# mpizenberg/visual-odometry-rs

Measured on AMD Instinct MI355X. Metric: frame-pairs/sec (640x480, 6 pyramid levels), higher is better.
Workload: dtype f32

## Files before the change

visual-odometry-rs_amd/csrc/kernels.hip:

```cpp
#include <hip/hip_runtime.h>

#include <algorithm>
#include <cstdint>
#include <cstdlib>

#include "device_common.h"
#include "engine.h"
#include "synth_scene.h"

namespace vors {

template <class T>
__global__ void transpose_kernel(const T* __restrict__ src, T* __restrict__ dst, int rows, int cols) {
    __shared__ T tile[32][33];
    const size_t base = (size_t)blockIdx.z * rows * cols;
    int sx = blockIdx.x * 32 + threadIdx.x;
    int sy = blockIdx.y * 32 + threadIdx.y;
    for (int j = 0; j < 32; j += 8)
        if (sx < rows && sy + j < cols) tile[threadIdx.y + j][threadIdx.x] = src[base + (size_t)(sy + j) * rows + sx];
    __syncthreads();
    int dx = blockIdx.y * 32 + threadIdx.x;
    int dy = blockIdx.x * 32 + threadIdx.y;
    for (int j = 0; j < 32; j += 8)
        if (dx < cols && dy + j < rows) dst[base + (size_t)(dy + j) * cols + dx] = tile[threadIdx.x][threadIdx.y + j];
// ... 315 lines not shown
                uint32_t k3 = (uint32_t)__builtin_amdgcn_update_dpp(0, (int)key, 0xff, 0xf, 0xf, true);
                {
                    uint32_t lo, hi;
                    lo = min(k0, k1); hi = max(k0, k1); k0 = lo; k1 = hi;
                    lo = min(k2, k3); hi = max(k2, k3); k2 = lo; k3 = hi;
                    lo = min(k0, k2); hi = max(k0, k2); k0 = lo; k2 = hi;
                    lo = min(k1, k3); hi = max(k1, k3); k1 = lo; k3 = hi;
                    lo = min(k1, k2); hi = max(k1, k2); k1 = lo; k2 = hi;
                }
                const uint32_t second = k2 >> 2, third = k1 >> 2;
                const bool keep2 = second > ((third + thresh) & 0xffffu);
                if (in && key >= k2) {
                    const bool best = key == k3;
                    const int dst = rl * NODES + offc + 2 * k + (best ? 0 : 1);
                    xy[dst] = (pvalid && (best || keep2)) ? ((uint32_t)cx | ((uint32_t)cy << 16)) : VORS_INVALID_XY;
                    gr[dst] = slim_pack_tg(tm, gx, gy);
                }
            }
        }
        kf_wave_sync();
    }

    {
        const int cap = 1 << (L - 1), off = cap - 1;
        for (int t = lane; t < KF_R * cap; t += 64) {
            const int rl = t >> (L - 1), k = t & (cap - 1);
            const uint32_t p = xy[rl * NODES + off + k];
            if (p != VORS_INVALID_XY) {
                const uint16_t dz = (depth + (size_t)pair * g.S0)[(p >> 16) * (unsigned)g.lv[0].cols + (p & 0xffffu)];
                if (dz == 0) {
                    xy[rl * NODES + off + k] = VORS_INVALID_XY;
                } else {
                    sd[rl * NODES + off + k] = g.depth_scale / (float)dz;
                    sv[rl * NODES + off + k] = g.idepth_variance;
                }
            }
        }
    }
    kf_wave_sync();
#pragma unroll
    for (int l = 1; l < L; ++l) {
        const int cap = 1 << (L - 1 - l);
        const int off = cap - 1, offc = 2 * cap - 1;
        for (int t = lane; t < KF_R * cap; t += 64) {
            const int rl = t >> (L - 1 - l), k = t & (cap - 1);
            const int c1 = rl * NODES + offc + 2 * k, c2 = c1 + 1, dst = rl * NODES + off + k;
            const bool k1 = xy[c1] != VORS_INVALID_XY, k2 = xy[c2] != VORS_INVALID_XY;
            if (k1 && k2) {
                const float d1 = sd[c1], v1 = sv[c1], d2 = sd[c2], v2 = sv[c2];
                const float sum = v1 + v2;
                sd[dst] = (d1 * v1 + d2 * v2) / sum;
                sv[dst] = sum;
            } else if (k1 || k2) {
                const int src = k1 ? c1 : c2;
                sd[dst] = sd[src];
                sv[dst] = sv[src];
            } else {
                xy[dst] = VORS_INVALID_XY;
            }
        }
        kf_wave_sync();
    }
    const int region = blockIdx.x * KF_WAVES + wave;
#pragma unroll
    for (int l = 0; l < L; ++l) {
        const int cap = 1 << (L - 1 - l), off = cap - 1;
        const int n_here = min(KF_R, max(0, n_roots - root0)) * cap;
        SlimRec* out = rec.stage + (size_t)pair * g.slots_total + g.lv[l].slot_off + (size_t)root0 * cap;
        int filled = 0;
        for (int base = 0; base < n_here; base += 64) {
            const int t = base + lane;
            const int rl = t >> (L - 1 - l), k = t & (cap - 1);
            const bool in = t < n_here;
            const uint32_t p = in ? xy[rl * NODES + off + k] : VORS_INVALID_XY;
            const bool valid = p != VORS_INVALID_XY;
            const unsigned long long m = __ballot(valid);
            const int before = __builtin_amdgcn_mbcnt_hi((unsigned)(m >> 32), __builtin_amdgcn_mbcnt_lo((unsigned)m, 0));
            if (valid) out[(unsigned)(filled + before)] = SlimRec{p, sd[rl * NODES + off + k], gr[rl * NODES + off + k]};
            filled += __popcll(m);
        }
        if (lane == 0) rec.region_cnt[((size_t)pair * VORS_MAX_LEVELS + l) * rec.n_regions + region] = filled;
    }
}

__global__ __launch_bounds__(256) void compact_regions_kernel(Geom g, Records rec) {
    __shared__ int s_cnt[256], s_pre[256], s_wave[4];
    __shared__ int s_base;
    const int pair = select_pair(g, blockIdx.y);
    if (pair < 0) return;
    const int lane = threadIdx.x & 63, wave = threadIdx.x >> 6;
    const int l_first = gridDim.x > 1 ? (int)blockIdx.x : 0, l_end = gridDim.x > 1 ? l_first + 1 : g.L;
    for (int l = l_first; l < l_end; ++l) {
        const int cap_r = rec.kf_r << (g.L - 1 - l);
        const int* cnt = rec.region_cnt + ((size_t)pair * VORS_MAX_LEVELS + l) * rec.n_regions;
        const size_t lvl0 = (size_t)pair * g.slots_total + g.lv[l].slot_off;
        const SlimRec* src = rec.stage + lvl0;
        SlimRec* dst = rec.S + lvl0;
        __syncthreads();
        if (threadIdx.x == 0) s_base = 0;
        __syncthreads();
        for (int tile = 0; tile < rec.n_regions; tile += 256) {
            const int r = tile + (int)threadIdx.x;
            const int mine = r < rec.n_regions ? cnt[r] : 0;
            int incl = mine;
#pragma unroll
            for (int o = 1; o < 64; o <<= 1) {
                const int v = __shfl_up(incl, o);
                if (lane >= o) incl += v;
            }
            if (lane == 63) s_wave[wave] = incl;
            __syncthreads();
            int pre = s_base + incl - mine;
            for (int w = 0; w < wave; ++w) pre += s_wave[w];
            s_cnt[threadIdx.x] = mine;
            s_pre[threadIdx.x] = pre;
            __syncthreads();
            const int n_tile = min(256, rec.n_regions - tile);
            const int cap_sh = __ffs(cap_r) - 1;
            for (int j = threadIdx.x; j < n_tile * cap_r; j += 256) {
                const int rr = j >> cap_sh, k = j & (cap_r - 1);
                if (k < s_cnt[rr]) dst[s_pre[rr] + k] = src[(size_t)(tile + rr) * cap_r + k];
            }
            __syncthreads();
            if (threadIdx.x == 255) s_base = pre + mine;
            __syncthreads();
        }
        if (threadIdx.x == 0) rec.n_used[(size_t)pair * VORS_MAX_LEVELS + l] = s_base;
    }
}

__device__ __forceinline__ void fuse_dso_mean(const float dv_in[4], const float vv_in[4], float* od, float* ov) {
    float sd = 0.f, sv = 0.f, single = 0.f;
    int n = 0;
#pragma unroll
    for (int m = 0; m < 4; ++m) {
        const bool known = vv_in[m] >= 0.f;
        const float prod = dv_in[m] * vv_in[m];
        sd += known ? prod : 0.f;
        sv += known ? vv_in[m] : 0.f;
        single = known ? dv_in[m] : single;
        n += known ? 1 : 0;
    }
    const float q = sd / sv;
    *od = n == 0 ? __builtin_nanf("") : (n == 1 ? single : q);
    *ov = n == 0 ? -1.0f : sv;
}
template <bool FAST>
__device__ __forceinline__ float idepth_of(float scale, uint32_t dz) {
    const float d = (float)dz;
    if (FAST) {
        const float rc = __builtin_amdgcn_rcpf(d);
        const float q = scale * rc;
        return fmaf(fmaf(-q, d, scale), rc, q);
    }
    return scale / d;
}
template <bool FAST>
__device__ __forceinline__ void fuse_depths(float scale, float var, const uint32_t dz[4], float* od, float* ov, int& n0) {
    float sd = 0.f, sv = 0.f, s1 = 0.f;
    int n = 0;
#pragma unroll
    for (int m = 0; m < 4; ++m) {
        const bool known = dz[m] != 0;
        const float d = known ? idepth_of<FAST>(scale, dz[m]) : 0.f;
        sd += d * var;
        sv += known ? var : 0.f;
        s1 += d;
        n += known ? 1 : 0;
    }
    n0 += n;
    const float q = sd / sv;
    *od = n == 0 ? __builtin_nanf("") : (n == 1 ? s1 : q);
    *ov = n == 0 ? -1.0f : sv;
}
__global__ void verify_idepth_kernel(float scale, int* mismatch) {
    const uint32_t dz = blockIdx.x * blockDim.x + threadIdx.x;
    if (dz == 0 || dz > 65535u) return;
    if (idepth_of<true>(scale, dz) != idepth_of<false>(scale, dz)) atomicExch(mismatch, 1);
}
bool verify_fast_idepth(float scale, hipStream_t s) {
    if (!(scale == scale) || !(fabsf(scale) < 1e30f) || !(fabsf(scale) > 1e-20f)) return false;
    int* flag = nullptr;
    if (hipMalloc(reinterpret_cast<void**>(&flag), sizeof(int)) != hipSuccess) return false;
    (void)hipMemsetAsync(flag, 0, sizeof(int), s);
    hipLaunchKernelGGL(verify_idepth_kernel, dim3(256), dim3(256), 0, s, scale, flag);
    int h = 1;
    const bool ok = hipMemcpyAsync(&h, flag, sizeof(int), hipMemcpyDeviceToHost, s) == hipSuccess && hipStreamSynchronize(s) == hipSuccess;
    (void)hipFree(flag);
    return ok && h == 0;
}
__device__ __forceinline__ void count_add(int* counter, int n) {
#pragma unroll
    for (int o = 32; o >= 1; o >>= 1) n += __shfl_xor(n, o);
    if ((threadIdx.x & 63) == 0 && n != 0) atomicAdd(counter, n);
}
template <bool FAST>
__global__ __launch_bounds__(256) void dense_idepth_level1_kernel(Geom g, const uint16_t* __restrict__ depth, Records rec) {
    const int pair = select_pair(g, blockIdx.y);
    if (pair < 0) return;
    const int t = blockIdx.x * blockDim.x + threadIdx.x;
    const int rows = g.lv[1].rows, cols = g.lv[1].cols;
    int n0 = 0, n1 = 0;
    if (t < rows * cols) {
        const int y = t / cols, x = t - y * cols;
        const int fr = g.lv[0].rows, fc = g.lv[0].cols;
        const uint16_t* p = depth + (size_t)pair * g.S0 + (size_t)(2 * y) * fc + 2 * x;
        const uint32_t dz[4] = {p[0], p[fc], p[1], p[fc + 1]};
        float od, ov;
        fuse_depths<FAST>(g.depth_scale, g.idepth_variance, dz, &od, &ov, n0);
        const bool last_x = x == cols - 1 && (fc & 1), last_y = y == rows - 1 && (fr & 1);
        if (last_x) n0 += (p[2] != 0) + (p[fc + 2] != 0);
        if (last_y) n0 += (p[2 * fc] != 0) + (p[2 * fc + 1] != 0);
        if (last_x && last_y) n0 += p[2 * fc + 2] != 0;
        const size_t slot = (size_t)pair * g.slots_total + g.lv[1].slot_off + t;
        rec.IZ[slot] = od;
        rec.V[slot] = ov;
        n1 = ov >= 0.f;
    }
    count_add(rec.n_used + (size_t)pair * VORS_MAX_LEVELS + 0, n0);
    count_add(rec.n_used + (size_t)pair * VORS_MAX_LEVELS + 1, n1);
}
template <bool FAST>
__global__ __launch_bounds__(256) void dense_idepth_level1_wide_kernel(Geom g, const uint16_t* __restrict__ depth, Records rec) {
    const int pair = select_pair(g, blockIdx.y);
    if (pair < 0) return;
    const int t0 = (blockIdx.x * blockDim.x + threadIdx.x) * 4;
    const int rows = g.lv[1].rows, cols = g.lv[1].cols;
    int n0 = 0, n1 = 0;
    if (t0 < rows * cols) {
        const int y = t0 / cols, x0 = t0 - y * cols;
        const int fr = g.lv[0].rows, fc = g.lv[0].cols;
        const uint16_t* p = depth + (size_t)pair * g.S0 + (size_t)(2 * y) * fc + 2 * x0;
        const uint4 r0 = *reinterpret_cast<const uint4*>(p), r1 = *reinterpret_cast<const uint4*>(p + fc);
        const uint32_t w0[4] = {r0.x, r0.y, r0.z, r0.w}, w1[4] = {r1.x, r1.y, r1.z, r1.w};
        float od[4], ov[4];
#pragma unroll
        for (int k = 0; k < 4; ++k) {
            const uint32_t dz[4] = {w0[k] & 0xffffu, w1[k] & 0xffffu, w0[k] >> 16, w1[k] >> 16};
            fuse_depths<FAST>(g.depth_scale, g.idepth_variance, dz, &od[k], &ov[k], n0);
            n1 += ov[k] >= 0.f;
        }
        if (y == rows - 1 && (fr & 1)) {
            const uint4 r2 = *reinterpret_cast<const uint4*>(p + 2 * fc);
            const uint32_t w2[4] = {r2.x, r2.y, r2.z, r2.w};
#pragma unroll
            for (int k = 0; k < 4; ++k) n0 += ((w2[k] & 0xffffu) != 0) + ((w2[k] >> 16) != 0);
        }
        const size_t slot = (size_t)pair * g.slots_total + g.lv[1].slot_off + t0;
        *reinterpret_cast<float4*>(rec.IZ + slot) = make_float4(od[0], od[1], od[2], od[3]);
        *reinterpret_cast<float4*>(rec.V + slot) = make_float4(ov[0], ov[1], ov[2], ov[3]);
    }
    count_add(rec.n_used + (size_t)pair * VORS_MAX_LEVELS + 0, n0);
    count_add(rec.n_used + (size_t)pair * VORS_MAX_LEVELS + 1, n1);
}
template <bool FAST>
__global__ __launch_bounds__(256) void dense_idepth_level12_kernel(Geom g, const uint16_t* __restrict__ depth, Records rec) {
    const int pair = select_pair(g, blockIdx.y);
    if (pair < 0) return;
    const int t = (blockIdx.x * blockDim.x + threadIdx.x) * 2;
    const int rows2 = g.lv[2].rows, cols2 = g.lv[2].cols;
    int n0 = 0, n1 = 0, n2 = 0;
    if (t < rows2 * cols2) {
        const int y2 = t / cols2, x2 = t - y2 * cols2;
        const int fc = g.lv[0].cols, c1 = g.lv[1].cols;
        const uint16_t* p = depth + (size_t)pair * g.S0 + (size_t)(4 * y2) * fc + 4 * x2;
        uint32_t w[4][4];
#pragma unroll
        for (int r = 0; r < 4; ++r) {
            const uint4 v = *reinterpret_cast<const uint4*>(p + (size_t)r * fc);
            w[r][0] = v.x;
            w[r][1] = v.y;
            w[r][2] = v.z;
            w[r][3] = v.w;
        }
        float od1[2][4], ov1[2][4];
#pragma unroll
        for (int i = 0; i < 2; ++i)
#pragma unroll
            for (int j = 0; j < 4; ++j) {
                const uint32_t top = w[2 * i][j], bot = w[2 * i + 1][j];
                const uint32_t dz[4] = {top & 0xffffu, bot & 0xffffu, top >> 16, bot >> 16};
                fuse_depths<FAST>(g.depth_scale, g.idepth_variance, dz, &od1[i][j], &ov1[i][j], n0);
                n1 += ov1[i][j] >= 0.f;
            }
        const size_t s1 = (size_t)pair * g.slots_total + g.lv[1].slot_off + (size_t)(2 * y2) * c1 + 2 * x2;
        *reinterpret_cast<float4*>(rec.IZ + s1) = make_float4(od1[0][0], od1[0][1], od1[0][2], od1[0][3]);
        *reinterpret_cast<float4*>(rec.IZ + s1 + c1) = make_float4(od1[1][0], od1[1][1], od1[1][2], od1[1][3]);
        float od[2], ov[2];
#pragma unroll
        for (int k = 0; k < 2; ++k) {
            const float dv2[4] = {od1[0][2 * k], od1[1][2 * k], od1[0][2 * k + 1], od1[1][2 * k + 1]};
            const float vv2[4] = {ov1[0][2 * k], ov1[1][2 * k], ov1[0][2 * k + 1], ov1[1][2 * k + 1]};
            fuse_dso_mean(dv2, vv2, &od[k], &ov[k]);
            n2 += ov[k] >= 0.f;
        }
        const size_t s2 = (size_t)pair * g.slots_total + g.lv[2].slot_off + t;
        *reinterpret_cast<float2*>(rec.IZ + s2) = make_float2(od[0], od[1]);
        *reinterpret_cast<float2*>(rec.V + s2) = make_float2(ov[0], ov[1]);
    }
    count_add(rec.n_used + (size_t)pair * VORS_MAX_LEVELS + 0, n0);
    count_add(rec.n_used + (size_t)pair * VORS_MAX_LEVELS + 1, n1);
    count_add(rec.n_used + (size_t)pair * VORS_MAX_LEVELS + 2, n2);
}
template <bool FAST>
__global__ __launch_bounds__(256) void dense_idepth_level123_kernel(Geom g, const uint16_t* __restrict__ depth, Records rec) {
    const int pair = select_pair(g, blockIdx.y);
    if (pair < 0) return;
    const int t = blockIdx.x * blockDim.x + threadIdx.x;
    const int cols3 = g.lv[3].cols;
    int n0 = 0, n1 = 0, n2 = 0, n3 = 0;
    if (t < g.lv[3].rows * cols3) {
        const int y3 = t / cols3, x3 = t - y3 * cols3;
        const int fc = g.lv[0].cols, c1 = g.lv[1].cols, c2 = g.lv[2].cols;
        const size_t base = (size_t)pair * g.slots_total;
        float od2[2][2], ov2[2][2];
        const uint16_t* p = depth + (size_t)pair * g.S0 + (size_t)(8 * y3) * fc + 8 * x3;
        uint4 v8[8];
#pragma unroll
        for (int r = 0; r < 8; ++r) v8[r] = *reinterpret_cast<const uint4*>(p + (size_t)r * fc);
#pragma unroll
        for (int h = 0; h < 2; ++h) {
            uint32_t w[4][4];
#pragma unroll
            for (int r = 0; r < 4; ++r) {
                const uint4 v = v8[4 * h + r];
                w[r][0] = v.x;
                w[r][1] = v.y;
                w[r][2] = v.z;
                w[r][3] = v.w;
            }
            float od1[2][4], ov1[2][4];
#pragma unroll
            for (int i = 0; i < 2; ++i)
#pragma unroll
                for (int j = 0; j < 4; ++j) {
                    const uint32_t top = w[2 * i][j], bot = w[2 * i + 1][j];
                    const uint32_t dz[4] = {top & 0xffffu, bot & 0xffffu, top >> 16, bot >> 16};
                    fuse_depths<FAST>(g.depth_scale, g.idepth_variance, dz, &od1[i][j], &ov1[i][j], n0);
                    n1 += ov1[i][j] >= 0.f;
                }
            const size_t s1 = base + g.lv[1].slot_off + (size_t)(4 * y3 + 2 * h) * c1 + 4 * x3;
            *reinterpret_cast<float4*>(rec.IZ + s1) = make_float4(od1[0][0], od1[0][1], od1[0][2], od1[0][3]);
            *reinterpret_cast<float4*>(rec.IZ + s1 + c1) = make_float4(od1[1][0], od1[1][1], od1[1][2], od1[1][3]);
#pragma unroll
            for (int k = 0; k < 2; ++k) {
                const float dv[4] = {od1[0][2 * k], od1[1][2 * k], od1[0][2 * k + 1], od1[1][2 * k + 1]};
                const float vv[4] = {ov1[0][2 * k], ov1[1][2 * k], ov1[0][2 * k + 1], ov1[1][2 * k + 1]};
                fuse_dso_mean(dv, vv, &od2[h][k], &ov2[h][k]);
                n2 += ov2[h][k] >= 0.f;
            }
            const size_t s2 = base + g.lv[2].slot_off + (size_t)(2 * y3 + h) * c2 + 2 * x3;
            *reinterpret_cast<float2*>(rec.IZ + s2) = make_float2(od2[h][0], od2[h][1]);
            *reinterpret_cast<float2*>(rec.V + s2) = make_float2(ov2[h][0], ov2[h][1]);
        }
        const float dv[4] = {od2[0][0], od2[1][0], od2[0][1], od2[1][1]};
        const float vv[4] = {ov2[0][0], ov2[1][0], ov2[0][1], ov2[1][1]};
        float od, ov;
        fuse_dso_mean(dv, vv, &od, &ov);
        n3 = ov >= 0.f;
        const size_t s3 = base + g.lv[3].slot_off + t;
        rec.IZ[s3] = od;
        rec.V[s3] = ov;
    }
    count_add(rec.n_used + (size_t)pair * VORS_MAX_LEVELS + 0, n0);
    count_add(rec.n_used + (size_t)pair * VORS_MAX_LEVELS + 1, n1);
    count_add(rec.n_used + (size_t)pair * VORS_MAX_LEVELS + 2, n2);
    count_add(rec.n_used + (size_t)pair * VORS_MAX_LEVELS + 3, n3);
}
__global__ __launch_bounds__(256) void dense_idepth_halve_kernel(Geom g, int l, Records rec) {
    const int pair = select_pair(g, blockIdx.y);
    if (pair < 0) return;
    const int t = blockIdx.x * blockDim.x + threadIdx.x;
    const int rows = g.lv[l].rows, cols = g.lv[l].cols;
    int n = 0;
    if (t < rows * cols) {
        const int y = t / cols, x = t - y * cols;
        const int fc = g.lv[l - 1].cols;
        const size_t cb = (size_t)pair * g.slots_total + g.lv[l - 1].slot_off + (size_t)(2 * y) * fc + 2 * x;
        const size_t idx[4] = {cb, cb + fc, cb + 1, cb + fc + 1};
        float dv[4], vv[4];
#pragma unroll
        for (int m = 0; m < 4; ++m) {
            dv[m] = rec.IZ[idx[m]];
            vv[m] = rec.V[idx[m]];
        }
        float od, ov;
        fuse_dso_mean(dv, vv, &od, &ov);
        const size_t slot = (size_t)pair * g.slots_total + g.lv[l].slot_off + t;
        rec.IZ[slot] = od;
        rec.V[slot] = ov;
        n = ov >= 0.f;
    }
    count_add(rec.n_used + (size_t)pair * VORS_MAX_LEVELS + l, n);
}
__global__ __launch_bounds__(256) void dense_materialize_kernel(Geom g, int l, int pair, const uint8_t* __restrict__ kf0,
                                                                 const uint8_t* __restrict__ kfu, const uint16_t* __restrict__ depth,
                                                                 Records rec, Records out) {
    const int t = blockIdx.x * blockDim.x + threadIdx.x;
    const int rows = g.lv[l].rows, cols = g.lv[l].cols;
    if (t >= rows * cols) return;
    const int y = t / cols, x = t - y * cols;
    float iz;
    bool valid;
    if (l == 0) {
        const uint16_t dz = depth[(size_t)pair * g.S0 + t];
        valid = dz != 0;
        iz = g.depth_scale / (float)dz;
    } else {
        iz = rec.IZ[(size_t)pair * g.slots_total + g.lv[l].slot_off + t];
        valid = !(iz != iz);
    }
    if (valid) {
        int gx, gy;
        grad_at(g, kf0, kfu, pair, l, x, y, &gx, &gy);
        write_record(out, t, g.lv[l].k, x, y, iz, gx, gy, level_ptr(g, kf0, kfu, pair, l)[t]);
    } else {
        write_empty(out, t);
    }
}
__global__ __launch_bounds__(256) void slim_materialize_kernel(Geom g, int l, int pair, Records rec, int n, Records out) {
    const int i = blockIdx.x * blockDim.x + threadIdx.x;
    if (i >= n) return;
    const SlimRec r = rec.S[(size_t)pair * g.slots_total + g.lv[l].slot_off + i];
    write_record(out, i, g.lv[l].k, (int)(r.xy & 0xffffu), (int)(r.xy >> 16), r.iz, slim_gx(r.tg), slim_gy(r.tg), (uint8_t)(r.tg & 0xff));
}
void launch_slim_materialize(const Geom& g, int l, int pair, Records rec, int n, Records out, hipStream_t s) {
    if (n <= 0) return;
    hipLaunchKernelGGL(slim_materialize_kernel, dim3((n + 255) / 256), dim3(256), 0, s, g, l, pair, rec, n, out);
}
void launch_dense_materialize(const Geom& g, int l, int pair, Pyramid kf, const uint16_t* depth, Records rec, Records out,
                              hipStream_t s) {
    hipLaunchKernelGGL(dense_materialize_kernel, dim3((g.lv[l].n_slots + 255) / 256), dim3(256), 0, s, g, l, pair, kf.level0, kf.upper,
                       depth, rec, out);
}

__global__ __launch_bounds__(64) void zero_ints_kernel(Geom g, int* __restrict__ base, int stride) {
    const int pair = select_pair(g, blockIdx.x);
    if (pair < 0) return;
    for (int i = threadIdx.x; i < stride; i += 64) base[(size_t)pair * stride + i] = 0;
}
void launch_zero_ints(const Geom& g, int* base, int stride, int n_pairs, hipStream_t s) {
    if (!g.sel_list) (void)hipMemsetAsync(base, 0, (size_t)n_pairs * stride * sizeof(int), s);
    else hipLaunchKernelGGL(zero_ints_kernel, dim3(n_pairs), dim3(64), 0, s, g, base, stride);
}

static int keyframe_roots_per_wave(const Geom& g) {
    static const int kf_r = getenv("VORS_KF_R") ? atoi(getenv("VORS_KF_R")) : 4;
    int r = kf_r >= 8 ? 8 : (kf_r >= 4 ? 4 : (kf_r >= 2 ? 2 : 1));
    while (r > 1 && (size_t)KF_WAVES * r * kf_nodes(g.L) * 16 > 64 * 1024) r >>= 1;
    return r;
}
void keyframe_region_geometry(const Geom& g, int* kf_r, int* n_regions) {
    const int r = keyframe_roots_per_wave(g), n_roots = g.root_rows * g.root_cols;
    *kf_r = r;
    *n_regions = ((n_roots + KF_WAVES * r - 1) / (KF_WAVES * r)) * KF_WAVES;
}
void launch_keyframe(const Geom& g, Pyramid kf, const uint16_t* depth, Records rec, int n_pairs, hipStream_t s) {
    if (g.mode == VORS_CANDIDATES_DENSE) {
        launch_zero_ints(g, rec.n_used, VORS_MAX_LEVELS, n_pairs, s);
        int next = 2;
        if (g.L >= 2) {
            const bool aligned = reinterpret_cast<uintptr_t>(depth) % 16 == 0;
            if (g.L >= 4 && aligned && g.lv[0].rows % 8 == 0 && g.lv[0].cols % 8 == 0 && !getenv("VORS_IDEPTH_LEVEL12")) {
                const dim3 grid((g.lv[3].n_slots + 255) / 256, n_pairs);
                if (g.fast_idepth) hipLaunchKernelGGL(dense_idepth_level123_kernel<true>, grid, dim3(256), 0, s, g, depth, rec);
                else hipLaunchKernelGGL(dense_idepth_level123_kernel<false>, grid, dim3(256), 0, s, g, depth, rec);
                next = 4;
            } else if (g.L >= 3 && aligned && g.lv[0].rows % 4 == 0 && g.lv[0].cols % 16 == 0) {
                if (g.fast_idepth) hipLaunchKernelGGL(dense_idepth_level12_kernel<true>, dim3((g.lv[2].n_slots / 2 + 255) / 256, n_pairs), dim3(256), 0, s, g, depth, rec);
                else hipLaunchKernelGGL(dense_idepth_level12_kernel<false>, dim3((g.lv[2].n_slots / 2 + 255) / 256, n_pairs), dim3(256), 0, s, g, depth, rec);
                next = 3;
            } else if (aligned && g.lv[0].cols % 8 == 0) {
                if (g.fast_idepth) hipLaunchKernelGGL(dense_idepth_level1_wide_kernel<true>, dim3((g.lv[1].n_slots / 4 + 255) / 256, n_pairs), dim3(256), 0, s, g, depth, rec);
                else hipLaunchKernelGGL(dense_idepth_level1_wide_kernel<false>, dim3((g.lv[1].n_slots / 4 + 255) / 256, n_pairs), dim3(256), 0, s, g, depth, rec);
            } else {
                if (g.fast_idepth) hipLaunchKernelGGL(dense_idepth_level1_kernel<true>, dim3((g.lv[1].n_slots + 255) / 256, n_pairs), dim3(256), 0, s, g, depth, rec);
                else hipLaunchKernelGGL(dense_idepth_level1_kernel<false>, dim3((g.lv[1].n_slots + 255) / 256, n_pairs), dim3(256), 0, s, g, depth, rec);
            }
        }
        for (int l = next; l < g.L; ++l)
            hipLaunchKernelGGL(dense_idepth_halve_kernel, dim3((g.lv[l].n_slots + 255) / 256, n_pairs), dim3(256), 0, s, g, l, rec);
    } else {
        const int r = rec.kf_r;
        dim3 grid(rec.n_regions / KF_WAVES, n_pairs);
        const size_t lds = (size_t)KF_WAVES * r * kf_nodes(g.L) * 16;
#ifndef VORS_KF_CONST_L
#define VORS_KF_CONST_L 1
#endif
        if (r == 8 && g.L == 6 && VORS_KF_CONST_L) hipLaunchKernelGGL((keyframe_sparse_kernel<8, 6>), grid, dim3(64 * KF_WAVES), lds, s, g, kf.level0, kf.upper, depth, rec);
        else if (r == 2 && g.L == 6 && VORS_KF_CONST_L) hipLaunchKernelGGL((keyframe_sparse_kernel<2, 6>), grid, dim3(64 * KF_WAVES), lds, s, g, kf.level0, kf.upper, depth, rec);
        else if (r == 8) hipLaunchKernelGGL((keyframe_sparse_kernel<8, 0>), grid, dim3(64 * KF_WAVES), lds, s, g, kf.level0, kf.upper, depth, rec);
        else if (r == 4 && g.L == 6 && VORS_KF_CONST_L) hipLaunchKernelGGL((keyframe_sparse_kernel<4, 6>), grid, dim3(64 * KF_WAVES), lds, s, g, kf.level0, kf.upper, depth, rec);
        else if (r == 4 && g.L == 7 && VORS_KF_CONST_L) hipLaunchKernelGGL((keyframe_sparse_kernel<4, 7>), grid, dim3(64 * KF_WAVES), lds, s, g, kf.level0, kf.upper, depth, rec);
        else if (r == 4) hipLaunchKernelGGL((keyframe_sparse_kernel<4, 0>), grid, dim3(64 * KF_WAVES), lds, s, g, kf.level0, kf.upper, depth, rec);
        else if (r == 2) hipLaunchKernelGGL((keyframe_sparse_kernel<2, 0>), grid, dim3(64 * KF_WAVES), lds, s, g, kf.level0, kf.upper, depth, rec);
        else hipLaunchKernelGGL((keyframe_sparse_kernel<1, 0>), grid, dim3(64 * KF_WAVES), lds, s, g, kf.level0, kf.upper, depth, rec);
        if (!ref_rank_from_regions(g, rec))
            hipLaunchKernelGGL(compact_regions_kernel, dim3(n_pairs <= 1024 ? g.L : 1, n_pairs), dim3(256), 0, s, g, rec);
    }
}

__global__ void verify_fastdiv_kernel(float d, float r, int* mismatch) {
    const uint32_t m = blockIdx.x * blockDim.x + threadIdx.x;
    if (m >= (1u << 23)) return;
    const FastDiv f{d, r, 1};
    const float x1 = __int_as_float((int)(0x3f800000u | m)), x2 = __int_as_float((int)(0x4b000000u | m));
    const bool bad = (div_uniform<true>(x1, f) != x1 / d) || (div_uniform<true>(-x1, f) != (-x1) / d) || (div_uniform<true>(x2, f) != x2 / d);
    if (bad) atomicExch(mismatch, 1);
}
bool verify_fastdiv(float d, float r, hipStream_t s) {
    if (!(d == d) || d == 0.0f || !(r == r) || fabsf(d) > 1e30f || fabsf(d) < 1e-30f) return false;
    int* flag = nullptr;
    if (hipMalloc(reinterpret_cast<void**>(&flag), sizeof(int)) != hipSuccess) return false;
    (void)hipMemsetAsync(flag, 0, sizeof(int), s);
    hipLaunchKernelGGL(verify_fastdiv_kernel, dim3((1u << 23) / 256), dim3(256), 0, s, d, r, flag);
    int h = 1;
    const bool ok = hipMemcpyAsync(&h, flag, sizeof(int), hipMemcpyDeviceToHost, s) == hipSuccess && hipStreamSynchronize(s) == hipSuccess;
    (void)hipFree(flag);
    return ok && h == 0;
}
__global__ void build_depth_lut_kernel(float depth_scale, float2* lut) {
    const int dz = blockIdx.x * blockDim.x + threadIdx.x;
    if (dz >= 65536) return;
    const float iz = depth_scale / (float)dz;
    lut[dz] = make_float2(iz, 1.0f / iz);
}
void launch_build_depth_lut(float depth_scale, float2* lut, hipStream_t s) {
    hipLaunchKernelGGL(build_depth_lut_kernel, dim3(256), dim3(256), 0, s, depth_scale, lut);
}

__global__ void synth_pairs_kernel(uint64_t seed0, int rows, int cols, vors_synth::CameraD cam, double motion_scale,
                                   int invalid_percent, uint8_t* kf_gray, uint16_t* kf_depth, uint8_t* cur_gray,
                                   uint16_t* cur_depth, float* gt_models7) {
    const int pair = blockIdx.y;
    const int t = blockIdx.x * blockDim.x + threadIdx.x;
    const uint64_t seed = seed0 + (uint64_t)pair;
    double xi[6];
    vors_synth::pair_twist(seed, motion_scale, xi);
    const vors_synth::RigidD m = vors_synth::se3_exp_d(xi);
    if (t == 0 && gt_models7) vors_synth::rigid_to_pose7(m, xi, gt_models7 + 7 * pair);
    if (t >= rows * cols) return;
    const int y = t / cols, x = t - y * cols;
    const size_t o = (size_t)pair * rows * cols + t;
    const double zero[6] = {0, 0, 0, 0, 0, 0};
    const vors_synth::RigidD id = vors_synth::se3_exp_d(zero);
    uint8_t gq;
    uint16_t dq;
    vors_synth::render_pixel(seed, 0, cam, id, x, y, invalid_percent, &gq, &dq);
    kf_gray[o] = gq;
    kf_depth[o] = dq;
    vors_synth::render_pixel(seed, 1, cam, m, x, y, invalid_percent, &gq, &dq);
    cur_gray[o] = gq;
    if (cur_depth) cur_depth[o] = dq;
}
void launch_synth_pairs(uint64_t seed0, int n_pairs, int rows, int cols, const double cam5[5], double motion_scale,
                        int invalid_percent, uint8_t* kf_gray, uint16_t* kf_depth, uint8_t* cur_gray, uint16_t* cur_depth,
                        float* gt_models7, hipStream_t s) {
    vors_synth::CameraD cam{cam5[0], cam5[1], cam5[2], cam5[3], cam5[4]};
    dim3 grid((rows * cols + 255) / 256, n_pairs);
    hipLaunchKernelGGL(synth_pairs_kernel, grid, dim3(256), 0, s, seed0, rows, cols, cam, motion_scale, invalid_percent, kf_gray,
                       kf_depth, cur_gray, cur_depth, gt_models7);
}

struct SynthFrame {
    uint64_t seed, salt;
    double xi[6];
};
__global__ void synth_frames_kernel(const SynthFrame* __restrict__ frames, int rows, int cols, vors_synth::CameraD cam, int invalid_percent,
                                    uint8_t* __restrict__ gray, uint16_t* __restrict__ depth) {
    const int f = blockIdx.y;
    const int t = blockIdx.x * blockDim.x + threadIdx.x;
    if (t >= rows * cols) return;
    const SynthFrame fr = frames[f];
    const vors_synth::RigidD m = vors_synth::se3_exp_d(fr.xi);
    const int y = t / cols, x = t - y * cols;
    const size_t o = (size_t)f * rows * cols + t;
    uint8_t gq;
    uint16_t dq;
    vors_synth::render_pixel(fr.seed, fr.salt, cam, m, x, y, invalid_percent, &gq, &dq);
    gray[o] = gq;
    depth[o] = dq;
}
void launch_synth_frames(const void* d_frames, int n_frames, int rows, int cols, const double cam5[5], int invalid_percent, uint8_t* gray,
                         uint16_t* depth, hipStream_t s) {
    vors_synth::CameraD cam{cam5[0], cam5[1], cam5[2], cam5[3], cam5[4]};
    dim3 grid((rows * cols + 255) / 256, n_frames);
    hipLaunchKernelGGL(synth_frames_kernel, grid, dim3(256), 0, s, static_cast<const SynthFrame*>(d_frames), rows, cols, cam, invalid_percent, gray,
                       depth);
}

__global__ __launch_bounds__(256) void trackers_advance_kernel(int n_seq, int* __restrict__ frame_counter, const float* __restrict__ out_poses7,
                                                               const vors_pair_stats* __restrict__ stats, float* __restrict__ cur_poses7,
                                                               float* __restrict__ kf_poses7, int32_t* __restrict__ kf_frame,
                                                               int* __restrict__ promo_list, int* __restrict__ promo_count) {
    __shared__ int s_wave[4];
    __shared__ int s_base;
    const int frame_index = *frame_counter + 1;
    if (threadIdx.x == 0) s_base = 0;
    __syncthreads();
    if (threadIdx.x == 0) *frame_counter = frame_index;
    const int lane = threadIdx.x & 63, wave = threadIdx.x >> 6;
    for (int s0 = 0; s0 < n_seq; s0 += 256) {
        const int s = s0 + (int)threadIdx.x;
        bool promote = false;
        if (s < n_seq) {
            promote = stats[s].change_keyframe != 0;
#pragma unroll
            for (int q = 0; q < 7; ++q) {
                const float v = out_poses7[7 * s + q];
                cur_poses7[7 * s + q] = v;
                if (promote) kf_poses7[7 * s + q] = v;
            }
            if (promote) kf_frame[s] = frame_index;
        }
        const unsigned long long m = __ballot(promote);
        if (lane == 0) s_wave[wave] = __popcll(m);
        __syncthreads();
        int before = s_base;
        for (int w = 0; w < wave; ++w) before += s_wave[w];
        if (promote) promo_list[before + __popcll(m & ((1ull << lane) - 1ull))] = s;
        __syncthreads();
        if (threadIdx.x == 0) s_base += s_wave[0] + s_wave[1] + s_wave[2] + s_wave[3];
        __syncthreads();
    }
    if (threadIdx.x == 0) *promo_count = s_base;
}
void launch_trackers_advance(int n_seq, int* frame_counter, const float* out_poses7, const vors_pair_stats* stats, float* cur_poses7,
                             float* kf_poses7, int32_t* kf_frame, int* promo_list, int* promo_count, hipStream_t s) {
    hipLaunchKernelGGL(trackers_advance_kernel, dim3(1), dim3(256), 0, s, n_seq, frame_counter, out_poses7, stats, cur_poses7, kf_poses7, kf_frame,
                       promo_list, promo_count);
}
__global__ __launch_bounds__(64) void tracker_pack_out_kernel(const float* __restrict__ pose7, const int32_t* __restrict__ status,
                                                              const int32_t* __restrict__ kf_frame, const vors_pair_stats* __restrict__ stats,
                                                              uint32_t* __restrict__ out) {
    const int t = threadIdx.x;
    constexpr int NS = (int)(sizeof(vors_pair_stats) / 4);
    if (t < 7) out[t] = __float_as_uint(pose7[t]);
    if (t == 7) out[7] = (uint32_t)status[0];
    if (t == 8) out[8] = (uint32_t)kf_frame[0];
    const uint32_t* sp = reinterpret_cast<const uint32_t*>(stats);
    for (int i = t; i < NS; i += 64) out[9 + i] = sp[i];
}
void launch_tracker_pack_out(const float* pose7, const int32_t* status, const int32_t* kf_frame, const vors_pair_stats* stats, void* out,
                             hipStream_t s) {
    hipLaunchKernelGGL(tracker_pack_out_kernel, dim3(1), dim3(64), 0, s, pose7, status, kf_frame, stats, static_cast<uint32_t*>(out));
}
__global__ __launch_bounds__(256) void promote_copy_kernel(Geom g, const uint8_t* __restrict__ src, size_t src_stride, uint8_t* __restrict__ dst,
                                                           size_t dst_stride, size_t bytes, int vec) {
    const int pair = select_pair(g, blockIdx.y);
    if (pair < 0) return;
    const uint8_t* sp = src + (size_t)pair * src_stride;
    uint8_t* dp = dst + (size_t)pair * dst_stride;
    const size_t t = ((size_t)blockIdx.x * blockDim.x + threadIdx.x) * 16;
    if (t >= bytes) return;
    if (vec && t + 16 <= bytes) {
        *reinterpret_cast<uint4*>(dp + t) = *reinterpret_cast<const uint4*>(sp + t);
    } else {
        for (size_t k = t; k < bytes && k < t + 16; ++k) dp[k] = sp[k];
    }
}
__global__ void identity_poses_kernel(float* __restrict__ a, float* __restrict__ b, int n) {
    const int i = blockIdx.x * blockDim.x + threadIdx.x;
    if (i < 7 * n) {
        const float v = (i % 7 == 6) ? 1.0f : 0.0f;
        a[i] = v;
        b[i] = v;
    }
}
void launch_identity_poses(float* a, float* b, int n, hipStream_t s) {
    hipLaunchKernelGGL(identity_poses_kernel, dim3((7 * n + 255) / 256), dim3(256), 0, s, a, b, n);
}
void launch_promote_copy(const Geom& g, const void* src, size_t src_stride, void* dst, size_t dst_stride, size_t bytes, int n_pairs,
                         hipStream_t s) {
    const int vec = (((uintptr_t)src | (uintptr_t)dst | src_stride | dst_stride) % 16 == 0) ? 1 : 0;
    hipLaunchKernelGGL(promote_copy_kernel, dim3((unsigned)((bytes + 4095) / 4096), n_pairs), dim3(256), 0, s, g, static_cast<const uint8_t*>(src),
                       src_stride, static_cast<uint8_t*>(dst), dst_stride, bytes, vec);
}
__global__ __launch_bounds__(256) void depth_weight_init_kernel(const uint16_t* __restrict__ depth, uint8_t* __restrict__ weight, size_t n, int vec) {
    const size_t i = ((size_t)blockIdx.x * 256 + threadIdx.x) * 16;
    if (i >= n) return;
    if (vec && i + 16 <= n) {
        const uint4 a = *reinterpret_cast<const uint4*>(depth + i), b = *reinterpret_cast<const uint4*>(depth + i + 8);
        const uint32_t d[8] = {a.x, a.y, a.z, a.w, b.x, b.y, b.z, b.w};
        uint32_t w[4];
#pragma unroll
        for (int k = 0; k < 4; ++k) {
            const uint32_t lo = d[2 * k], hi = d[2 * k + 1];
            w[k] = ((lo & 0xffffu) ? 1u : 0u) | ((lo >> 16) ? 0x100u : 0u) | ((hi & 0xffffu) ? 0x10000u : 0u) | ((hi >> 16) ? 0x1000000u : 0u);
        }
        *reinterpret_cast<uint4*>(weight + i) = make_uint4(w[0], w[1], w[2], w[3]);
    } else {
        for (size_t k = i; k < n && k < i + 16; ++k) weight[k] = depth[k] ? 1 : 0;
    }
}
void launch_depth_weight_init(const uint16_t* depth, uint8_t* weight, size_t n, hipStream_t s) {
    const int vec = (((uintptr_t)depth | (uintptr_t)weight) % 16 == 0) ? 1 : 0;
    hipLaunchKernelGGL(depth_weight_init_kernel, dim3((unsigned)((n + 4095) / 4096)), dim3(256), 0, s, depth, weight, n, vec);
}

}
```

Baseline: 347,900.

## Fuse dense idepth pyramid levels 1-5 into one kernel via LDS reduction

Replaces the level-1..3 idepth kernel with one that also computes levels 4 and 5. Threads are regrouped into 4x4 tiles of level-3 pixels so one block reduces through shared memory, which removes the separate halve-kernel launches and their global reloads. It also stops writing the variance (V) buffer for intermediate levels, packs two counters per wave reduction to halve atomics, and uses packed u16 min instructions for counting known depths. This adds block syncs and a single-wave tail for levels 4-5, and relies on weight-sum identities that are checked on the host.

Measured after the change: 350,100 (median of 6 runs). About the same (+0.6%).

```diff
diff --git a/visual-odometry-rs_amd/csrc/kernels.hip b/visual-odometry-rs_amd/csrc/kernels.hip
--- a/visual-odometry-rs_amd/csrc/kernels.hip
+++ b/visual-odometry-rs_amd/csrc/kernels.hip
@@ -641,18 +641,87 @@
     count_add(rec.n_used + (size_t)pair * VORS_MAX_LEVELS + 1, n1);
     count_add(rec.n_used + (size_t)pair * VORS_MAX_LEVELS + 2, n2);
 }
+struct IdepthPx {
+    float d, w;
+    int known;
+};
+__device__ __forceinline__ int min1(int n) {
+    int r;
+    asm("v_min_u32 %0, 1, %1" : "=v"(r) : "v"(n));
+    return r;
+}
+__device__ __forceinline__ uint32_t min1_u16x2(uint32_t packed) {
+    uint32_t r;
+    asm("v_pk_min_u16 %0, %1, %2" : "=v"(r) : "v"(packed), "v"(0x00010001u));
+    return r;
+}
+__device__ __forceinline__ IdepthPx fuse_known(const IdepthPx& a, const IdepthPx& b, const IdepthPx& c, const IdepthPx& d) {
+    float sd = 0.f, sw = 0.f;
+    sd += fmaxf(a.d * a.w, 0.f);
+    sw += a.w;
+    sd += fmaxf(b.d * b.w, 0.f);
+    sw += b.w;
+    sd += fmaxf(c.d * c.w, 0.f);
+    sw += c.w;
+    sd += fmaxf(d.d * d.w, 0.f);
+    sw += d.w;
+    const float single = fmaxf(fmaxf(a.d, b.d), fmaxf(c.d, d.d));
+    const int n = (a.known + b.known) + (c.known + d.known);
+    const float q = sd / sw;
+    IdepthPx o;
+    o.d = n == 0 ? __builtin_nanf("") : (n == 1 ? single : q);
+    o.w = sw;
+    o.known = min1(n);
+    return o;
+}
 template <bool FAST>
-__global__ __launch_bounds__(256) void dense_idepth_level123_kernel(Geom g, const uint16_t* __restrict__ depth, Records rec) {
+__device__ __forceinline__ IdepthPx fuse_depth_words(float scale, float var, uint32_t top, uint32_t bot, int& n0) {
+    const uint32_t dz[4] = {top & 0xffffu, bot & 0xffffu, top >> 16, bot >> 16};
+    float dd[4], sd = 0.f;
+#pragma unroll
+    for (int m = 0; m < 4; ++m) {
+        if (FAST) dd[m] = fmaxf(idepth_of<true>(scale, dz[m]), 0.f);
+        else dd[m] = dz[m] != 0 ? idepth_of<false>(scale, dz[m]) : 0.f;
+        sd += dd[m] * var;
+    }
+    const uint32_t kw = min1_u16x2(top) + min1_u16x2(bot);
+    const int n = (int)((kw & 0xffffu) + (kw >> 16));
+    n0 += n;
+    const float single = fmaxf(fmaxf(dd[0], dd[1]), fmaxf(dd[2], dd[3]));
+    IdepthPx o;
+    o.w = (float)n * var;
+    const float q = sd / o.w;
+    o.d = n == 0 ? __builtin_nanf("") : (n == 1 ? single : q);
+    o.known = min1(n);
+    return o;
+}
+__device__ __forceinline__ void count_add2(int* counter_a, int* counter_b, int packed) {
+#pragma unroll
+    for (int o = 32; o >= 1; o >>= 1) packed += __shfl_xor(packed, o);
+    if ((threadIdx.x & 63) == 0) {
+        if (packed & 0xffff) atomicAdd(counter_a, packed & 0xffff);
+        if (packed >> 16) atomicAdd(counter_b, packed >> 16);
+    }
+}
+template <bool FAST, bool V_TOP>
+__global__ __launch_bounds__(256) void dense_idepth_level1to5_kernel(Geom g, const uint16_t* __restrict__ depth, Records rec) {
+    __shared__ float s_d3[256], s_w3[256], s_d4[64], s_w4[64];
     const int pair = select_pair(g, blockIdx.y);
     if (pair < 0) return;
-    const int t = blockIdx.x * blockDim.x + threadIdx.x;
-    const int cols3 = g.lv[3].cols;
-    int n0 = 0, n1 = 0, n2 = 0, n3 = 0;
-    if (t < g.lv[3].rows * cols3) {
-        const int y3 = t / cols3, x3 = t - y3 * cols3;
+    const int lane = threadIdx.x & 63, wave = threadIdx.x >> 6;
+    const int gx = lane & 3, gq = (lane >> 2) & 3, gy = lane >> 4;
+    const int rows3 = g.lv[3].rows, cols3 = g.lv[3].cols;
+    const int gcols = (cols3 + 3) >> 2, n_groups = gcols * ((rows3 + 3) >> 2);
+    const int grp = blockIdx.x * 16 + wave * 4 + gq;
+    const int grp_y = grp / gcols, grp_x = grp - grp_y * gcols;
+    const int x3 = 4 * grp_x + gx, y3 = 4 * grp_y + gy;
+    const size_t base = (size_t)pair * g.slots_total;
+    int* const n_used = rec.n_used + (size_t)pair * VORS_MAX_LEVELS;
+    int n0 = 0, n1 = 0, n2 = 0;
+    IdepthPx px3 = {__builtin_nanf(""), 0.f, 0};
+    if (grp < n_groups && x3 < cols3 && y3 < rows3) {
         const int fc = g.lv[0].cols, c1 = g.lv[1].cols, c2 = g.lv[2].cols;
-        const size_t base = (size_t)pair * g.slots_total;
-        float od2[2][2], ov2[2][2];
+        IdepthPx px2[2][2];
         const uint16_t* p = depth + (size_t)pair * g.S0 + (size_t)(8 * y3) * fc + 8 * x3;
         uint4 v8[8];
 #pragma unroll
@@ -668,43 +737,69 @@
                 w[r][2] = v.z;
                 w[r][3] = v.w;
             }
-            float od1[2][4], ov1[2][4];
+            IdepthPx px1[2][4];
 #pragma unroll
             for (int i = 0; i < 2; ++i)
 #pragma unroll
                 for (int j = 0; j < 4; ++j) {
-                    const uint32_t top = w[2 * i][j], bot = w[2 * i + 1][j];
-                    const uint32_t dz[4] = {top & 0xffffu, bot & 0xffffu, top >> 16, bot >> 16};
-                    fuse_depths<FAST>(g.depth_scale, g.idepth_variance, dz, &od1[i][j], &ov1[i][j], n0);
-                    n1 += ov1[i][j] >= 0.f;
+                    px1[i][j] = fuse_depth_words<FAST>(g.depth_scale, g.idepth_variance, w[2 * i][j], w[2 * i + 1][j], n0);
+                    n1 += px1[i][j].known;
                 }
             const size_t s1 = base + g.lv[1].slot_off + (size_t)(4 * y3 + 2 * h) * c1 + 4 * x3;
-            *reinterpret_cast<float4*>(rec.IZ + s1) = make_float4(od1[0][0], od1[0][1], od1[0][2], od1[0][3]);
-            *reinterpret_cast<float4*>(rec.IZ + s1 + c1) = make_float4(od1[1][0], od1[1][1], od1[1][2], od1[1][3]);
+            *reinterpret_cast<float4*>(rec.IZ + s1) = make_float4(px1[0][0].d, px1[0][1].d, px1[0][2].d, px1[0][3].d);
+            *reinterpret_cast<float4*>(rec.IZ + s1 + c1) = make_float4(px1[1][0].d, px1[1][1].d, px1[1][2].d, px1[1][3].d);
 #pragma unroll
             for (int k = 0; k < 2; ++k) {
-                const float dv[4] = {od1[0][2 * k], od1[1][2 * k], od1[0][2 * k + 1], od1[1][2 * k + 1]};
-                const float vv[4] = {ov1[0][2 * k], ov1[1][2 * k], ov1[0][2 * k + 1], ov1[1][2 * k + 1]};
-                fuse_dso_mean(dv, vv, &od2[h][k], &ov2[h][k]);
-                n2 += ov2[h][k] >= 0.f;
+                px2[h][k] = fuse_known(px1[0][2 * k], px1[1][2 * k], px1[0][2 * k + 1], px1[1][2 * k + 1]);
+                n2 += px2[h][k].known;
             }
             const size_t s2 = base + g.lv[2].slot_off + (size_t)(2 * y3 + h) * c2 + 2 * x3;
-            *reinterpret_cast<float2*>(rec.IZ + s2) = make_float2(od2[h][0], od2[h][1]);
-            *reinterpret_cast<float2*>(rec.V + s2) = make_float2(ov2[h][0], ov2[h][1]);
-        }
-        const float dv[4] = {od2[0][0], od2[1][0], od2[0][1], od2[1][1]};
-        const float vv[4] = {ov2[0][0], ov2[1][0], ov2[0][1], ov2[1][1]};
-        float od, ov;
-        fuse_dso_mean(dv, vv, &od, &ov);
-        n3 = ov >= 0.f;
-        const size_t s3 = base + g.lv[3].slot_off + t;
-        rec.IZ[s3] = od;
-        rec.V[s3] = ov;
-    }
-    count_add(rec.n_used + (size_t)pair * VORS_MAX_LEVELS + 0, n0);
-    count_add(rec.n_used + (size_t)pair * VORS_MAX_LEVELS + 1, n1);
-    count_add(rec.n_used + (size_t)pair * VORS_MAX_LEVELS + 2, n2);
-    count_add(rec.n_used + (size_t)pair * VORS_MAX_LEVELS + 3, n3);
+            *reinterpret_cast<float2*>(rec.IZ + s2) = make_float2(px2[h][0].d, px2[h][1].d);
+        }
+        px3 = fuse_known(px2[0][0], px2[1][0], px2[0][1], px2[1][1]);
+        rec.IZ[base + g.lv[3].slot_off + (size_t)y3 * cols3 + x3] = px3.d;
+    }
+    count_add2(n_used + 0, n_used + 1, n0 + (n1 << 16));
+    count_add2(n_used + 2, n_used + 3, n2 + (px3.known << 16));
+    if (g.L < 5) return;
+    const int slot3 = (wave * 4 + gq) * 16 + gy * 4 + gx;
+    s_d3[slot3] = px3.d;
+    s_w3[slot3] = px3.w;
+    __syncthreads();
+    const int worker = (blockIdx.x + blockIdx.y) & 3;
+    if (wave == worker) {
+        const int cx = lane & 1, cy = (lane >> 1) & 1, q = lane >> 2;
+        const int grp4 = blockIdx.x * 16 + q, grp4_y = grp4 / gcols, grp4_x = grp4 - grp4_y * gcols;
+        const int x4 = 2 * grp4_x + cx, y4 = 2 * grp4_y + cy;
+        const int a = q * 16 + 8 * cy + 2 * cx;
+        const IdepthPx ca = {s_d3[a], s_w3[a], s_w3[a] > 0.f}, cb = {s_d3[a + 4], s_w3[a + 4], s_w3[a + 4] > 0.f};
+        const IdepthPx cc = {s_d3[a + 1], s_w3[a + 1], s_w3[a + 1] > 0.f}, cd = {s_d3[a + 5], s_w3[a + 5], s_w3[a + 5] > 0.f};
+        const IdepthPx px4 = fuse_known(ca, cb, cc, cd);
+        const bool in4 = grp4 < n_groups && x4 < g.lv[4].cols && y4 < g.lv[4].rows;
+        if (in4) rec.IZ[base + g.lv[4].slot_off + (size_t)y4 * g.lv[4].cols + x4] = px4.d;
+        s_d4[lane] = px4.d;
+        s_w4[lane] = px4.w;
+        count_add(n_used + 4, in4 ? px4.known : 0);
+    }
+    if (g.L < 6) return;
+    __syncthreads();
+    if (wave == worker) {
+        int n5 = 0;
+        if (lane < 16) {
+            const int grp5 = blockIdx.x * 16 + lane, y5 = grp5 / gcols, x5 = grp5 - y5 * gcols;
+            const int a = 4 * lane;
+            const IdepthPx ca = {s_d4[a], s_w4[a], s_w4[a] > 0.f}, cb = {s_d4[a + 2], s_w4[a + 2], s_w4[a + 2] > 0.f};
+            const IdepthPx cc = {s_d4[a + 1], s_w4[a + 1], s_w4[a + 1] > 0.f}, cd = {s_d4[a + 3], s_w4[a + 3], s_w4[a + 3] > 0.f};
+            const IdepthPx px5 = fuse_known(ca, cb, cc, cd);
+            if (grp5 < n_groups && x5 < g.lv[5].cols && y5 < g.lv[5].rows) {
+                const size_t s5 = base + g.lv[5].slot_off + (size_t)y5 * g.lv[5].cols + x5;
+                rec.IZ[s5] = px5.d;
+                if (V_TOP) rec.V[s5] = px5.known ? px5.w : -1.0f;
+                n5 = px5.known;
+            }
+        }
+        count_add(n_used + 5, n5);
+    }
 }
 __global__ __launch_bounds__(256) void dense_idepth_halve_kernel(Geom g, int l, Records rec) {
     const int pair = select_pair(g, blockIdx.y);
@@ -794,17 +889,27 @@
     *kf_r = r;
     *n_regions = ((n_roots + KF_WAVES * r - 1) / (KF_WAVES * r)) * KF_WAVES;
 }
+static bool dense_idepth_fused_forms_ok(const Geom& g) {
+    const volatile float w = g.idepth_variance;
+    const volatile float w2 = w + w, w3 = w2 + w, w4 = w3 + w, m3 = 3.0f * w, m4 = 4.0f * w;
+    return g.depth_scale > 0.f && w > 0.f && w4 < 3.0e38f && w3 == m3 && w4 == m4;
+}
 void launch_keyframe(const Geom& g, Pyramid kf, const uint16_t* depth, Records rec, int n_pairs, hipStream_t s) {
     if (g.mode == VORS_CANDIDATES_DENSE) {
         launch_zero_ints(g, rec.n_used, VORS_MAX_LEVELS, n_pairs, s);
         int next = 2;
         if (g.L >= 2) {
             const bool aligned = reinterpret_cast<uintptr_t>(depth) % 16 == 0;
-            if (g.L >= 4 && aligned && g.lv[0].rows % 8 == 0 && g.lv[0].cols % 8 == 0 && !getenv("VORS_IDEPTH_LEVEL12")) {
-                const dim3 grid((g.lv[3].n_slots + 255) / 256, n_pairs);
-                if (g.fast_idepth) hipLaunchKernelGGL(dense_idepth_level123_kernel<true>, grid, dim3(256), 0, s, g, depth, rec);
-                else hipLaunchKernelGGL(dense_idepth_level123_kernel<false>, grid, dim3(256), 0, s, g, depth, rec);
-                next = 4;
+            if (g.L >= 4 && aligned && g.lv[0].rows % 8 == 0 && g.lv[0].cols % 8 == 0 && dense_idepth_fused_forms_ok(g) &&
+                !getenv("VORS_IDEPTH_LEVEL12")) {
+                const int n_groups = ((g.lv[3].cols + 3) / 4) * ((g.lv[3].rows + 3) / 4);
+                const dim3 grid((n_groups + 15) / 16, n_pairs);
+                const bool v_top = g.L > 6;
+                if (g.fast_idepth && v_top) hipLaunchKernelGGL((dense_idepth_level1to5_kernel<true, true>), grid, dim3(256), 0, s, g, depth, rec);
+                else if (g.fast_idepth) hipLaunchKernelGGL((dense_idepth_level1to5_kernel<true, false>), grid, dim3(256), 0, s, g, depth, rec);
+                else if (v_top) hipLaunchKernelGGL((dense_idepth_level1to5_kernel<false, true>), grid, dim3(256), 0, s, g, depth, rec);
+                else hipLaunchKernelGGL((dense_idepth_level1to5_kernel<false, false>), grid, dim3(256), 0, s, g, depth, rec);
+                next = std::min(g.L, 6);
             } else if (g.L >= 3 && aligned && g.lv[0].rows % 4 == 0 && g.lv[0].cols % 16 == 0) {
                 if (g.fast_idepth) hipLaunchKernelGGL(dense_idepth_level12_kernel<true>, dim3((g.lv[2].n_slots / 2 + 255) / 256, n_pairs), dim3(256), 0, s, g, depth, rec);
                 else hipLaunchKernelGGL(dense_idepth_level12_kernel<false>, dim3((g.lv[2].n_slots / 2 + 255) / 256, n_pairs), dim3(256), 0, s, g, depth, rec);
```
